# DarlingHang/st-nerf

Hardware: AMD Instinct MI355X
Metric: rendered rays/s (and ray-samples/s) per GPU, 1080p x 128-sample layered render (higher is better)
Workload: dtype f32 (operands split into 3 bf16 pieces, 6 bf16 MFMA terms per product, f32 accumulate); 1 GPU; taekwondo-1080p-64+64; precision=bf16x3, height=1080, width=1920, performer_layers=2, coarse_samples=64, fine_samples=64, parallelism=1 GPU, whole view

## Files before the change

### st-nerf_amd/csrc/mlp_bf16x3.h

```cpp
#pragma once
#include "mlp_common.h"

namespace stnerf {

constexpr int BX_CHUNK = 1024;
constexpr int BX_UNIT = 3 * BX_CHUNK;
constexpr int BX_SLOT = 8 * BX_UNIT;
constexpr int BX_RING = 4;
constexpr int BX_CONST_SPACE = 3072;
constexpr int BX_CONST_MOTION = 1024;
constexpr int BXC_B = 0, BXC_B_DEEP = 1792, BXC_W_SIGMA = 2048, BXC_W_RGB2 = 2304;
constexpr int BXM_B = 0, BXM_W_OUT = 640;

struct BxLayout {
    int64_t f32_floats;
    int64_t consts_off;
    int64_t stream_off;
    int32_t n_slots;
    int64_t total_bytes;
};

__host__ __device__ inline int bx_space_slots(bool deep) {
    return (2 * 4 + 5 * 2 * 16 + 2 * 20 + 16 + (deep ? 16 : 0)) / 2;
}
__host__ __device__ inline int bx_motion_slots() { return (6 + 4 * 8) / 2; }

__host__ __device__ inline BxLayout bx_layout(int kind) {
    BxLayout B;
    const bool space = STNERF_NET_IS_SPACE(kind);
    B.f32_floats = space ? space_layout(STNERF_NET_USES_TIME(kind), STNERF_NET_IS_DEEP(kind)).total : motion_layout().total;
    B.consts_off = (B.f32_floats * 4 + 1023) & ~int64_t(1023);
    B.stream_off = B.consts_off + (space ? BX_CONST_SPACE : BX_CONST_MOTION) * 4;
    B.n_slots = space ? bx_space_slots(STNERF_NET_IS_DEEP(kind)) : bx_motion_slots();
    B.total_bytes = B.stream_off + (int64_t)B.n_slots * BX_SLOT;
    return B;
}

constexpr int BXD_CONST = 1024;
constexpr int BXD_W_SIGMA = 0, BXD_W_RGB2 = 256;
__host__ __device__ inline int bxd_slots(bool with_dpos) { return 8 + 6 * 16 + (with_dpos ? 8 : 0); }

__host__ __device__ inline int bx_kmap_hidden(int t, int h, int j) { return 32 * (t >> 1) + 8 * (2 * (t & 1) + (j >> 2)) + 4 * h + (j & 3); }
__host__ __device__ inline int bx_kmap_enc(int t, int h, int j) { return 16 * t + 8 * h + j; }

struct StageArgs;
struct StoreTapArgs;
struct StageRowsArgs;
int launch_bf16x3_stage_rows(const StageArgs& a, const StageRowsArgs& r, bool deep_rgb, int cus, hipStream_t stream);
int launch_bf16x3_stage(const StageArgs& a, bool deep_rgb, int cus, hipStream_t stream);
int launch_bf16x3_stage_store(const StageArgs& a, const StoreTapArgs& t, int cus, hipStream_t stream);

struct MotionBxArgs {
    const float* net;
    const int32_t* ray_list;
    const int32_t* ray_count;
    int64_t n_rays;
    int32_t ns;
    int32_t flags;
    float* xyz;
    int64_t xyz_ray_stride;
    const float* times;
    int64_t times_ray_stride;
    const int32_t* slots;
    int64_t slot_ray_stride;
    uint32_t* queue;
    int64_t stream_off;
};
int launch_bf16x3_motion(const MotionBxArgs& a, int cus, hipStream_t stream);

}
```

### st-nerf_amd/csrc/mlp_bf16x3_core.h

```cpp
#pragma once
#include <type_traits>

#include "mlp_wave_common.h"
#include "mlp_bf16x3.h"

namespace stnerf {

using bf16x8 = __attribute__((ext_vector_type(8))) __bf16;
using bf16x2 = __attribute__((ext_vector_type(2))) __bf16;
using u32x4 = __attribute__((ext_vector_type(4))) unsigned;

constexpr int BX_LDS_RING = BX_RING * BX_SLOT;
constexpr int BX_LDS_ENC = WV_NW * WV_ENC_FLOATS * 4;
constexpr int BX_LDS_CONST = (BX_CONST_SPACE + BX_CONST_MOTION) * 4;
constexpr int BX_LDS = BX_LDS_RING + BX_LDS_ENC + BX_LDS_CONST + 16 + STNERF_MAX_LAYERS * 8 + (STNERF_MAX_LAYERS + 1) * 4 + 12;
static_assert(BX_LDS <= 160 * 1024, "bf16x3 stage kernel: LDS budget");

#define BX_SB() __builtin_amdgcn_sched_barrier(0)

#ifdef STNERF_BX_PROF
struct BxProf {
    unsigned long long t, acc[16];
};
#define BXP_PARAM , BxProf& bp
// ... 194 lines not shown
        BX_SB();
    }
    if (FIRST && BIG0) {
        const f32x16 z = {0.f, 0.f, 0.f, 0.f, 0.f, 0.f, 0.f, 0.f, 0.f, 0.f, 0.f, 0.f, 0.f, 0.f, 0.f, 0.f};
        big = mfma_bf16(cur.p[0], b0, z);
    } else {
        big = mfma_bf16(cur.p[0], b0, big);
    }
    if (DMA0 >= 0) {
        BX_SB();
        dma_chunk<DMA0 < 0 ? 0 : DMA0 + 2>(*dma);
    }
    if constexpr (!std::is_same<Hook, NoHook>::value) {
        BX_SB();
        hook->template at<U, 2>();
    }
    BX_SB();
}

template <int ST = 0>
__device__ __forceinline__ void slot_turn(Ctx& cx, Dma& d) {
    if constexpr (ST > 0) {
        if (cx.st_on)
            BX_VMCNT(6 + ST);
        else
            BX_VMCNT(6);
    } else {
        BX_VMCNT(6);
    }
    __builtin_amdgcn_s_barrier();
    dma_begin(cx, d);
    BX_SB();
}
__device__ __forceinline__ void slot_done(Ctx& cx) {
    cx.gc += 1;
    cx.rcur = cx.rnext;
    cx.rnext = cx.rnext + (((cx.gc + 1) & (BX_RING - 1)) == 0 ? BX_SLOT - BX_RING * BX_SLOT : BX_SLOT);
}

template <bool FIRST, bool BIG0 = false, class Hook = NoHook, int ST = 0>
__device__ __forceinline__ void slot(Ctx& cx, f32x16 (&big)[4], f32x16 (&small)[4], const bf16x8& k0p0, const bf16x8& k0p1,
                                     const bf16x8& k0p2, const bf16x8& k1p0, const bf16x8& k1p1, const bf16x8& k1p2, Hook* hook = nullptr) {
    unit<0, FIRST, BIG0, -1, Hook>(cx, big[0], small[0], k0p0, k0p1, k0p2, nullptr, hook);
    unit<1, FIRST, BIG0, -1, Hook>(cx, big[1], small[1], k0p0, k0p1, k0p2, nullptr, hook);
    unit<2, FIRST, BIG0, -1, Hook>(cx, big[2], small[2], k0p0, k0p1, k0p2, nullptr, hook);
    unit<3, FIRST, BIG0, -1, Hook>(cx, big[3], small[3], k0p0, k0p1, k0p2, nullptr, hook);
    unit<4, false, false, -1, Hook>(cx, big[0], small[0], k1p0, k1p1, k1p2, nullptr, hook);
    unit<5, false, false, -1, Hook>(cx, big[1], small[1], k1p0, k1p1, k1p2, nullptr, hook);
    Dma d;
    slot_turn<ST>(cx, d);
    unit<6, false, false, 0, Hook>(cx, big[2], small[2], k1p0, k1p1, k1p2, &d, hook);
    unit<7, false, false, 3, Hook>(cx, big[3], small[3], k1p0, k1p1, k1p2, &d, hook);
    slot_done(cx);
}

template <int KS0, int NSLOT, bool FIRST, bool BIG0 = false, int ST = 0>
__device__ __forceinline__ void pass_act(Ctx& cx, f32x16 (&big)[4], f32x16 (&small)[4], const bf16x8 (&act)[3][16]) {
#pragma unroll
    for (int sl = 0; sl < NSLOT; ++sl) {
        const int k = KS0 + 2 * sl;
        if (sl == 0)
            slot<FIRST, BIG0, NoHook, ST>(cx, big, small, act[0][k], act[1][k], act[2][k], act[0][k + 1], act[1][k + 1], act[2][k + 1]);
        else if (sl == 1)
            slot<false, false, NoHook, ST>(cx, big, small, act[0][k], act[1][k], act[2][k], act[0][k + 1], act[1][k + 1], act[2][k + 1]);
        else
            slot<false>(cx, big, small, act[0][k], act[1][k], act[2][k], act[0][k + 1], act[1][k + 1], act[2][k + 1]);
    }
}

__device__ __forceinline__ void load_c(f32x16 (&big)[4], const float* v128, int lane) {
    const float4* b4 = reinterpret_cast<const float4*>(v128) + (lane >> 5);
#pragma unroll
    for (int fb = 0; fb < 4; ++fb)
#pragma unroll
        for (int q = 0; q < 4; ++q) {
            const float4 b = b4[fb * 8 + 2 * q];
            big[fb][4 * q + 0] = b.x;
            big[fb][4 * q + 1] = b.y;
            big[fb][4 * q + 2] = b.z;
            big[fb][4 * q + 3] = b.w;
            BX_SB();
        }
}
__device__ __forceinline__ void load_c_block(f32x16& bigfb, const float* v128, int fb, int lane) {
    const float4* b4 = reinterpret_cast<const float4*>(v128) + (lane >> 5);
#pragma unroll
    for (int q = 0; q < 4; ++q) {
        const float4 b = b4[fb * 8 + 2 * q];
        bigfb[4 * q + 0] = b.x;
        bigfb[4 * q + 1] = b.y;
        bigfb[4 * q + 2] = b.z;
        bigfb[4 * q + 3] = b.w;
    }
}
__device__ __forceinline__ float out_relu(const f32x16& big, const f32x16& small, int i) { return relu_bits(big[i] + small[i]); }

struct Park {
    float v[64];
};
__device__ __forceinline__ void park_put(float& dst, float v) { asm("v_accvgpr_write_b32 %0, %1" : "=a"(dst) : "v"(v)); }
__device__ __forceinline__ float park_get(const float& src) {
    float v;
    asm("v_accvgpr_read_b32 %0, %1" : "=v"(v) : "a"(src));
    return v;
}

// ... 213 lines not shown
    for (int t = 0; t < STEPS; ++t) {
        float v[8];
#pragma unroll
        for (int qq = 0; qq < 2; ++qq) {
            float4 x = make_float4(0.f, 0.f, 0.f, 0.f);
            if (4 * t + 2 + qq < NQ) {
                x = e4[(4 * t + 2 * h + qq) * WV_ROWS + c];
            } else if (4 * t + qq < NQ) {
                const float4 y = e4[(4 * t + qq) * WV_ROWS + c];
                x.x = h == 0 ? y.x : 0.f;
                x.y = h == 0 ? y.y : 0.f;
                x.z = h == 0 ? y.z : 0.f;
                x.w = h == 0 ? y.w : 0.f;
            }
            v[4 * qq + 0] = x.x;
            v[4 * qq + 1] = x.y;
            v[4 * qq + 2] = x.z;
            v[4 * qq + 3] = x.w;
        }
        enc_tap(t, v);
        split8(v, act[0][t], act[1][t], act[2][t]);
        BX_SB();
    }
}

template <int INST = 0>
__device__ __forceinline__ void motion_bx(Ctx& cx, const float* net, const float* cm, float* encw, float (&p)[3], float tv, int flags,
                                          int lane, f32x16 (&big)[4], f32x16 (&small)[4], bf16x8 (&act)[3][16] BXP_PARAM) {
    const MotionLayout L = motion_layout();
    load_c(big, cm + BXM_B, lane);
    encode_motion(encw, lane, p, tv, flags);
    wave_lds_sync();
    enc_to_act<6, WV_ENC_QUADS>(encw, lane, act);
    BXP(BXP_MOTION_ENC);
    pass_act<0, 3, true>(cx, big, small, act);
    BXP(BXP_MOTION_PASS);
#pragma unroll 1
    for (int li = 1; li <= 4; ++li) {
        finish_act<0>(big, small, act, cm + BXM_B + 128 * li, lane);
        BXP(BXP_MOTION_FIN);
        pass_act<0, 4, true>(cx, big, small, act);
        BXP(BXP_MOTION_PASS);
    }
    float fl[3];
    head3(big, small, cm + BXM_W_OUT, net + L.b_out, lane, fl);
#pragma unroll
    for (int c3 = 0; c3 < 3; ++c3) p[c3] = p[c3] + fl[c3];
    BXP(BXP_MOTION_FIN);
}

template <bool DEEP, class Mid, class Tap>
__device__ __forceinline__ float4 space_bx(Ctx& cx, const float* net, const bool use_time, const float* cs, float* encw, const float (&p)[3],
                                           const float* __restrict__ raybias, int32_t ray, int lane, f32x16 (&big)[4], f32x16 (&small)[4],
                                           bf16x8 (&act)[3][16], Mid mid, const Tap& tap BXP_PARAM) {
    const SpaceLayout L = space_layout(use_time, DEEP);
    const int h = lane >> 5;
    constexpr int ST = Tap::on ? BX_TAP_PARK : 0;
    Park pk;
    load_c(big, cs + BXC_B, lane);
    encode_pos(encw, lane, p);
    wave_lds_sync();
    if constexpr (Tap::on) {
        const bool valid = tap_valid(tap, lane);
        float4* dst = reinterpret_cast<float4*>(tap_row(tap, TAP_PE, 4 * h, lane));
        enc_to_act<4, 16>(encw, lane, act, [&](int t, const float (&v)[8]) {
            if (valid) {
                dst[4 * t] = make_float4(v[0], v[1], v[2], v[3]);
                dst[4 * t + 1] = make_float4(v[4], v[5], v[6], v[7]);
            }
        });
    } else {
        enc_to_act<4, 16>(encw, lane, act);
    }
    BXP(BXP_PE);
    pass_act<0, 2, true, false, Tap::on ? BX_TAP_PE : 0>(cx, big, small, act);
    BXP(BXP_PASS);
    finish_park(big, small, pk, cs + BXC_B + 128, lane, tap, 0, 0);
    BXP(BXP_PARK);
    pass_act<0, 2, true, false, ST>(cx, big, small, act);
    BXP(BXP_PASS);
    unpark_act(pk, act);
    BXP(BXP_ACT);
    finish_park(big, small, pk, cs + BXC_B + 256, lane, tap, 0, 128);
    BXP(BXP_PARK);
#define BX_INLINED(call)                           \
    do {                                           \
        if constexpr (Tap::on) {                   \
            [[clang::always_inline]] call;         \
        } else {                                   \
            call;                                  \
        }                                          \
    } while (0)
    auto pe_slots = [&]() {
        const float4* e4 = reinterpret_cast<const float4*>(encw);
#pragma unroll
        for (int sl = 0; sl < 2; ++sl) {
            bf16x8 pe[2][3];
#pragma unroll
            for (int t = 0; t < 2; ++t) {
                float v[8];
#pragma unroll
                for (int qq = 0; qq < 2; ++qq) {
                    const float4 x = e4[(4 * (2 * sl + t) + 2 * h + qq) * WV_ROWS + (lane & 31)];
                    v[4 * qq + 0] = x.x;
                    v[4 * qq + 1] = x.y;
                    v[4 * qq + 2] = x.z;
                    v[4 * qq + 3] = x.w;
                }
                split8(v, pe[t][0], pe[t][1], pe[t][2]);
            }
            slot<false>(cx, big, small, pe[0][0], pe[0][1], pe[0][2], pe[1][0], pe[1][1], pe[1][2]);
        }
    };
    auto layer = [&](int li, auto with_pe) {
        pass_a_unpark<false, ST>(cx, big, small, act, pk);
        pass_act<8, 4, false>(cx, big, small, act);
        if constexpr (decltype(with_pe)::value) BX_INLINED(pe_slots());
        BXP(BXP_PASS);
        finish_park(big, small, pk, cs + BXC_B + 256 * li + 128, lane, tap, li, 0);
        BXP(BXP_PARK);
        pass_b_unpark<ST>(cx, big, small, act, pk);
        if constexpr (decltype(with_pe)::value) BX_INLINED(pe_slots());
        BXP(BXP_PASS);
    };
    auto layer_end = [&](int li) {
        finish_park(big, small, pk, li < 6 ? cs + BXC_B + 256 * (li + 1) : nullptr, lane, tap, li, 128);
        BXP(BXP_PARK);
    };
#pragma unroll 1
    for (int li = 1; li <= 3; ++li) {
        BX_INLINED(layer(li, std::false_type{}));
        BX_INLINED(layer_end(li));
    }
    BX_INLINED(layer(4, std::true_type{}));
    BX_INLINED(layer_end(4));
    float sigma = 0.f;
#pragma unroll 1
    for (int li = 5; li <= 6; ++li) {
        BX_INLINED(layer(li, std::false_type{}));
        if (li == 6) {
            mid();
            sigma = sigma_head(big, small, pk, cs + BXC_W_SIGMA, net[L.b_sigma], lane);
            BXP(BXP_SIGMA);
        }
        BX_INLINED(layer_end(li));
    }
#undef BX_INLINED
    pass_a_unpark<true, ST>(cx, big, small, act, pk);
    pass_act<8, 3, false>(cx, big, small, act);
    BXP(BXP_PASS);
    {
        float4 crow[4][4];
        const float* row = raybias + (int64_t)ray * 128 + 4 * h;
#pragma unroll
        for (int fb = 0; fb < 4; ++fb)
#pragma unroll
            for (int q = 0; q < 4; ++q) crow[fb][q] = *reinterpret_cast<const float4*>(row + fb * 32 + 8 * q);
        pass_act<14, 1, false>(cx, big, small, act);
        BXP(BXP_PASS);
#pragma unroll
        for (int fb = 0; fb < 4; ++fb) {
#pragma unroll
            for (int q = 0; q < 4; ++q) {
                big[fb][4 * q + 0] = (big[fb][4 * q + 0] + small[fb][4 * q + 0]) + crow[fb][q].x;
                big[fb][4 * q + 1] = (big[fb][4 * q + 1] + small[fb][4 * q + 1]) + crow[fb][q].y;
                big[fb][4 * q + 2] = (big[fb][4 * q + 2] + small[fb][4 * q + 2]) + crow[fb][q].z;
                big[fb][4 * q + 3] = (big[fb][4 * q + 3] + small[fb][4 * q + 3]) + crow[fb][q].w;
            }
#pragma unroll
            for (int i = 0; i < 16; ++i) small[fb][i] = 0.f;
            BX_SB();
        }
    }
    if constexpr (Tap::on) finish_park<false>(big, small, pk, nullptr, lane, tap, 7, 0);
    if constexpr (DEEP) {
#pragma unroll 1
        for (int i = 0; i < 2; ++i) {
            finish_act<0>(big, small, act, cs + BXC_B_DEEP + 128 * i, lane);
            pass_act<0, 4, true>(cx, big, small, act);
        }
    }
    float rgb[3];
    head3(big, small, cs + BXC_W_RGB2, net + L.b_rgb2, lane, rgb);
    BXP(BXP_RGB_TAIL);
    return make_float4(rgb[0], rgb[1], rgb[2], sigma);
}

__device__ __forceinline__ void ring_init(Ctx& cx, char* ring, int wave, int lane) {
    cx.ring = ring;
    cx.wave = wave;
    cx.lane = lane;
    cx.gi = 0;
    cx.gc = 0;
    cx.rcur = (uint32_t)(uintptr_t)ring + (uint32_t)lane * 16u;
    cx.rnext = cx.rcur + BX_SLOT;
}
__device__ __forceinline__ void ring_start(Ctx& cx) {
    dma_issue(cx);
    dma_issue(cx);
    dma_issue(cx);
// ... 12 lines not shown
```

### st-nerf_amd/csrc/mlp_bf16x3_stage_kernel.h

```cpp
#pragma once
#include "mlp_bf16x3_core.h"

namespace stnerf {

#ifdef STNERF_BX_PROF
static __device__ unsigned long long g_bxphase[16];
#endif

__device__ __forceinline__ bool tap_wave_stores(const BxStoreTap& tap, const StoreTapArgs& t) {
    return (uint32_t)(tap.wave * WV_ROWS) < tap.nrows && t.bits != nullptr;
}
__device__ __forceinline__ BxNoTap make_bx_tap(const NoTapArgs&, uint32_t, int64_t, int) { return BxNoTap(); }
__device__ __forceinline__ BxNoTap make_bx_tap(const StageRowsArgs&, uint32_t, int64_t, int) { return BxNoTap(); }
__device__ __forceinline__ BxStoreTap make_bx_tap(const StoreTapArgs& t, uint32_t item, int64_t rows, int wave) {
    const int64_t left = rows - (int64_t)item * WV_ITEM;
    return BxStoreTap{&t, item * (uint32_t)WV_ITEM, (uint32_t)(left < WV_ITEM ? left : WV_ITEM), wave};
}

template <bool DEEP, class TapArgs>
__global__ __launch_bounds__(WV_THREADS, 1) void STNERF_STAGE_KERNEL(StageArgs a, TapArgs targs) {
    constexpr bool TAP = std::is_same<TapArgs, StoreTapArgs>::value;
    constexpr bool ROWS = std::is_same<TapArgs, StageRowsArgs>::value;
    extern __shared__ __attribute__((aligned(16))) char smem_bx[];
    const int tid = threadIdx.x;
// ... 122 lines not shown
    }
    Ctx cx;
    ring_init(cx, ring, wave, lane);
    cx.st_on = false;
    segs_of(it0, cx.seg[0], cx.seg[1]);
    segs_of(it1, cx.seg[2], cx.seg[3]);
    cx.idle = cx.seg[1].p;
    ring_start(cx);
    int par = 0;
    f32x16 big[4], small[4];
    bf16x8 act[3][16];
#ifdef STNERF_BX_PROF
    BxProf bp;
    for (int i = 0; i < 16; ++i) bp.acc[i] = 0;
    bp.t = clock64();
#endif
    while (it0 < total) {
        uint32_t pending = 0;
        if (tid == 0) pending = atomicAdd(a.queue, 1u);
        RowRef rr_next;
        uint32_t next_ray = 0;
        if constexpr (TAP) {
            const int64_t row = (int64_t)it1 * WV_ITEM + wave * WV_ROWS + (lane & 31);
            if (row < a.n_rays * a.ns) next_ray = (uint32_t)row / (uint32_t)a.ns;
        } else {
            row_of(it1, rr_next);
        }
        const StageLayer& ly = a.layer[slot_of(it0)];
        {
            const char* sc = reinterpret_cast<const char*>(ly.space) + (sp_kind_stream[ly.use_time ? 1 : 0] - BX_CONST_SPACE * 4) + lane * 16;
            auto d = (__attribute__((address_space(3))) char*)(cs);
#pragma unroll
            for (int i = 0; i < 3; ++i)
                __builtin_amdgcn_global_load_lds(sc + (wave + 4 * i) * BX_CHUNK, (__attribute__((address_space(3))) void*)(d + (wave + 4 * i) * BX_CHUNK), 16, 0, 0);
            if (ly.motion) {
                const char* mc = reinterpret_cast<const char*>(ly.motion) + (mo_stream - BX_CONST_MOTION * 4) + lane * 16;
                auto dm = (__attribute__((address_space(3))) char*)(cm);
                __builtin_amdgcn_global_load_lds(mc + wave * BX_CHUNK, (__attribute__((address_space(3))) void*)(dm + wave * BX_CHUNK), 16, 0, 0);
            }
        }
        float p[3];
#pragma unroll
        for (int c3 = 0; c3 < 3; ++c3) p[c3] = cur.p[c3];
        BX_VMCNT(0);
        __builtin_amdgcn_s_barrier();
        BXP(BXP_TOP);
        int ln = lane;
        asm volatile("" : "+v"(ln));
        if constexpr (!TAP) {
            if (ly.motion) motion_bx(cx, ly.motion, cm, encw, p, cur.tv, ly.motion_flags, ln, big, small, act BXP_ARG);
        }
        const auto tap = make_bx_tap(targs, it0, a.n_rays * a.ns, wave);
        if constexpr (TAP) cx.st_on = tap_wave_stores(tap, targs);
        float4 o = space_bx<DEEP>(cx, ly.space, ly.use_time != 0, cs, encw, p, ly.raybias, cur.ray, ln, big, small, act,
                                  [&]() {
                                      if constexpr (TAP) {
                                          const int64_t row = (int64_t)it1 * WV_ITEM + wave * WV_ROWS + (lane & 31);
                                          rr_next.valid = row < a.n_rays * a.ns;
                                          rr_next.ray = next_ray;
                                          rr_next.k = (int)((uint32_t)row - next_ray * (uint32_t)a.ns);
                                      }
                                      fetch(it1, rr_next, nxt);
                                  }, tap BXP_ARG);
        if constexpr (TAP) {
            const int64_t row = (int64_t)it0 * WV_ITEM + wave * WV_ROWS + (lane & 31);
            cur.raw_off = (int64_t)cur.ray * a.raw_ray_stride + 4 * (row - (int64_t)cur.ray * a.ns);
        }
        if (cur.valid && lane < 32) {
            if (a.sigmoid_rgb) {
                o.x = __builtin_amdgcn_rcpf(1.f + __builtin_amdgcn_exp2f(o.x * -1.44269504088896340736f));
                o.y = __builtin_amdgcn_rcpf(1.f + __builtin_amdgcn_exp2f(o.y * -1.44269504088896340736f));
                o.z = __builtin_amdgcn_rcpf(1.f + __builtin_amdgcn_exp2f(o.z * -1.44269504088896340736f));
            }
            *reinterpret_cast<float4*>(ly.raw + cur.raw_off) = o;
        }
        if (tid == 0) qslot[par] = pending;
        __syncthreads();
        const uint32_t it2 = __builtin_amdgcn_readfirstlane(qslot[par]);
        par ^= 1;
        it0 = it1;
        it1 = it2;
        cur = nxt;
        cx.seg[0] = cx.seg[2];
        cx.seg[1] = cx.seg[3];
        segs_of(it1, cx.seg[2], cx.seg[3]);
        BXP(BXP_END);
#ifdef STNERF_BX_PROF
        bp.acc[BXP_ITEMS] += 1;
#endif
    }
    BX_VMCNT(0);
#ifdef STNERF_BX_PROF
    if (lane == 0)
        for (int i = 0; i < 16; ++i) atomicAdd(&g_bxphase[i], bp.acc[i]);
#endif
}

}
```

### st-nerf_amd/csrc/mlp_stage.h

```cpp
#pragma once
#include <type_traits>

#include "mlp_common.h"

namespace stnerf {

struct StageLayer {
    const float* space;
    const float* motion;
    const int32_t* ray_list;
    const int32_t* ray_count;
    const float* xyz;
    float* raw;
    const float* times;
    int32_t use_time;
    int32_t motion_flags;
    const float* raybias;
};

struct StageArgs {
    StageLayer layer[STNERF_MAX_LAYERS];
    int32_t n_layers, ns;
    int64_t n_rays;
    int64_t xyz_ray_stride, raw_ray_stride, dirs_ray_stride, times_ray_stride;
    const float* dirs;
    uint32_t* queue;
    int32_t sigmoid_rgb;
    float* dbg;
    int32_t dbg_stage;
};

__device__ __forceinline__ int64_t layer_rows(const int32_t* ray_count, int64_t n_rays, int ns) {
    int64_t cnt = n_rays;
    if (ray_count) {
        const int64_t c = *ray_count;
        cnt = c < cnt ? c : cnt;
    }
    return cnt * ns;
}
__device__ __forceinline__ int64_t layer_rows(const StageLayer& ly, int64_t n_rays, int ns) { return layer_rows(ly.ray_count, n_rays, ns); }

struct RowRef {
    int64_t ray;
    int k;
    bool valid;
};
__device__ __forceinline__ RowRef locate_row(const int32_t* ray_list, int64_t row, int64_t rows, int ns) {
    RowRef r{0, 0, row < rows};
    if (r.valid) {
        const int64_t slot = row / ns;
        r.k = (int)(row - slot * ns);
        r.ray = ray_list ? (int64_t)ray_list[slot] : slot;
    }
    return r;
}

__device__ __forceinline__ float lerp_enc(bool frac, float om, float wgt, float va, float vb) {
    return frac ? om * va + wgt * vb : va;
}

struct NoTapArgs {};
constexpr int TAP_PE = 100;
struct StoreTapArgs {
    float* buf[8];
    int32_t ld[8];
    float* pe;
    int32_t ld_pe;
    uint32_t* bits;
    int64_t bits_stride;
};
// ... 23 lines not shown
```

### st-nerf_amd/csrc/pipeline.hip

```cpp
#include <math.h>
#include <stdlib.h>
#include <string.h>

#include "common.h"
#include "mlp_bf16x3.h"

using namespace stnerf;

namespace {

struct Carve {
    char* base;
    int64_t off, cap;
    template <class T>
    T* take(int64_t count) {
        off = (off + 255) & ~int64_t(255);
        T* p = reinterpret_cast<T*>(base + off);
        off += count * (int64_t)sizeof(T);
        return p;
    }
};

struct Plan {
    int64_t t_c, xyz_c, raw_c, w_c, slots, t_f, xyz_f, raw_f, list, count, flags, raybias;
// ... 336 lines not shown
            STNERF_REQUIRE(((uintptr_t)e.raw_coarse & 15) == 0 && (p->only_coarse || ((uintptr_t)e.raw_fine & 15) == 0),
                           "render_rays: layer cache buffers of layer %d must be 16-byte aligned", i);
            STNERF_REQUIRE(e.capacity >= 0, "render_rays: layer cache entry %d with a negative capacity", i);
            (e.mode == STNERF_LAYER_CACHE_REUSE ? lreuse : lcap) |= 1u << i;
        }
    }
    call->lcap = lcap;
    call->lreuse = lreuse;
    call->term = 0;
    if (flagged && !p->only_coarse)
        for (int i = 0; i < l; ++i)
            if (o.terminate[i] && (i == 0 ? cache_mode == STNERF_BKGD_CACHE_OFF : p->shown[i] != 0 && !((lcap | lreuse) >> i & 1))) call->term |= 1u << i;
    if (o.occ) {
        const int orc = check_occupancy_table(o.occ, l, "render_rays");
        if (orc) return orc;
        STNERF_REQUIRE(((uintptr_t)o.counts & 7) == 0, "render_rays: occupancy counts must be 8-byte aligned");
    }
    return STNERF_OK;
}

int launch_sequence(RENDER_PARAMS, const stnerf_render_options& o, const Call& c, const Plan& pl, const Workspace& w, stnerf_stream_t stream) {
    const int l = p->l, n1 = p->n1, n2 = p->n2, S = n1 + n2, rs = p->ray_stride;
    const bool cached = c.cache_mode == STNERF_BKGD_CACHE_REUSE;
    const uint32_t lcap = c.lcap, lreuse = c.lreuse, term = c.term;
    const int64_t row_cap = c.rows.row_cap;
    hipStream_t st = as_stream(stream);
    int rc;

    rc = stnerf_sample_coarse_rot(rays, n, rs, boxes, box_ray_stride, l, n1, jitter, p->seed, p->ray_index_base,
                                  p->ray_index_stripe, p->ray_index_period,
                                  p->has_edits ? p->edits_coarse : nullptr, p->pivot, o.rot, w.t_c, w.xyz_c, mask, stream);
    if (rc) return rc;
    if (o.occ) {
        rc = stnerf_occupancy_cull(w.xyz_c, n, l, n1, o.occ, mask, o.counts, stream);
        if (rc) return rc;
    }
    if (hipMemsetAsync(w.ray_count, 0, sizeof(int32_t) * pl.count, st) != hipSuccess) {
        set_error("render_rays: hipMemsetAsync failed");
        return STNERF_ELAUNCH;
    }
    rc = stnerf_compact_rays(mask, n, l, w.ray_list, w.ray_count, stream);
    if (rc) return rc;

    uint32_t reuse = 0;
    if (p->precision == 3 && !p->only_coarse && p->use_deform_time) {
        const char* sw = getenv("STNERF_MOTION_REUSE");
        if (!(sw && sw[0] == '0'))
            for (int i = 1; i < l; ++i)
                if (p->shown[i] && !w.row_list[i] && !(lreuse >> i & 1) && (!p->has_edits || memcmp(&p->edits_coarse[i], &p->edits_fine[i], sizeof(stnerf_layer_edit)) == 0))
                    reuse |= 1u << i;
    }
    uint32_t* motion_queue = reinterpret_cast<uint32_t*>(w.ray_count + STNERF_MAX_LAYERS + 2);

    auto stage = [&](float* xyz, float* raw, int ns, bool fine, uint32_t moved) -> int {
        const int64_t xs = (int64_t)l * ns * 3, ws_ = (int64_t)l * ns * 4;
        if (p->precision == 0 || p->precision == 3) {
            stnerf_stage_layer sl[STNERF_MAX_LAYERS];
            stnerf_stage_rows sr[STNERF_MAX_LAYERS];
            memset(sr, 0, sizeof(sr));
            int ns_l = 0;
            bool any_list = false;
            for (int pass = 0; pass < 2; ++pass) {
                for (int i = cached ? 1 : 0; i < l; ++i) {
                    if (i > 0 && (!p->shown[i] || (lreuse >> i & 1))) continue;
                    const bool deform = i == 0 ? p->bkgd_use_deform_time != 0 : p->use_deform_time != 0;
                    if ((pass == 0) != deform) continue;
                    const bool timed = (i > 0 ? 1 : p->bkgd_use_space_time) && p->use_space_time;
                    stnerf_stage_layer& e = sl[ns_l++];
                    e.space = i == 0 ? (fine ? nets->bkgd_fine : nets->bkgd) : (fine ? nets->space_fine[i] : nets->space[i]);
                    e.motion = deform && !(moved >> i & 1) ? nets->motion[i] : nullptr;
                    e.ray_list = i == 0 ? nullptr : w.ray_list + (int64_t)i * n;
                    e.ray_count = i == 0 ? nullptr : w.ray_count + i;
                    e.xyz = xyz + (int64_t)i * ns * 3;
                    e.raw = raw + (int64_t)i * ns * 4;
                    e.times = (timed || deform) ? rays + (p->retiming ? 6 + i : 6) : nullptr;
                    e.use_time = timed ? 1 : 0;
                    e.motion_flags = i == 0 ? STNERF_MOTION_PLAIN_TIME : 0;
                    e.rotation = o.rot ? o.rot + i : nullptr;
                    const bool culled = o.samples && o.samples[i];
                    if (i == 0 && c.bg) {
                        const bool stop = fine && (term & 1);
                        const int r1 = stnerf_background_rows(n, e.xyz, xs, ns, o.bkgd_grid, stop ? w.t_f : nullptr, (int64_t)l * ns, stop ? w.t_stop : nullptr,
                                                              e.raw, ws_, w.row_list[0], row_cap, w.row_count, o.bkgd_counts, stream);
                        if (r1) return r1;
                    } else if (fine && (term >> i & 1)) {
                        const int r1 = stnerf_visibility_rows(e.ray_list, e.ray_count, n, i, e.xyz, xs, w.t_f + (int64_t)i * ns, (int64_t)l * ns, w.t_stop, ns,
                                                              culled ? o.occ + i : nullptr, e.raw, ws_, w.row_list[i], row_cap, w.row_count + i,
                                                              o.visibility_counts, stream);
                        if (r1) return r1;
                    } else if (culled) {
                        const int r1 = stnerf_occupancy_rows(e.ray_list, e.ray_count, n, i, e.xyz, xs, ns, o.occ + i, e.raw, ws_, w.row_list[i], row_cap,
                                                             w.row_count + i, o.sample_counts, stream);
                        if (r1) return r1;
                    } else {
                        continue;
                    }
                    sr[ns_l - 1].row_list = w.row_list[i];
                    sr[ns_l - 1].row_count = w.row_count + i;
                    any_list = true;
                }
            }
            if (ns_l == 0) return STNERF_OK;
            set_launch_tag(fine ? 1 : 0);
            const int r2 = stnerf_mlp_stage_rows(sl, any_list ? sr : nullptr, ns_l, n, ns, rays + 3, rs, rs, xs, ws_,
                                                 (p->deep_rgb ? STNERF_STAGE_DEEP_RGB : 0) | STNERF_STAGE_SIGMOID_RGB | (p->precision == 3 ? STNERF_STAGE_BF16X3 : 0),
                                                 reinterpret_cast<uint32_t*>(w.ray_count + STNERF_MAX_LAYERS + (fine ? 1 : 0)), w.ray_bias, stream);
            set_launch_tag(-1);
            return r2;
        }
        for (int i = cached ? 1 : 0; i < l; ++i) {
            if (i == 0 ? !p->bkgd_use_deform_time : !p->use_deform_time) continue;
            if (i > 0 && (!p->shown[i] || (lreuse >> i & 1))) continue;
            set_launch_tag(i);
            const float* times = rays + (p->retiming ? 6 + i : 6);
            const int32_t* lst = i == 0 ? nullptr : w.ray_list + (int64_t)i * n;
            const int32_t* cnt = i == 0 ? nullptr : w.ray_count + i;
            const int flags = STNERF_MOTION_ADD_TO_XYZ | (i == 0 ? STNERF_MOTION_PLAIN_TIME : 0);
            const int r2 = stnerf_motionnet_fwd(nets->motion[i], n, ns, lst, cnt, xyz + (int64_t)i * ns * 3, xs, times,
                                                      rs, nullptr, 0, flags, stream);
            if (r2) return r2;
        }
        for (int i = cached ? 1 : 0; i < l; ++i) {
            if (i > 0 && (!p->shown[i] || (lreuse >> i & 1))) continue;
            set_launch_tag(i);
            const void* net = i == 0 ? (fine ? nets->bkgd_fine : nets->bkgd) : (fine ? nets->space_fine[i] : nets->space[i]);
            const bool timed = (i > 0 ? 1 : p->bkgd_use_space_time) && p->use_space_time;
            const int kind = timed ? (p->deep_rgb ? STNERF_NET_SPACE_TIME_DEEP : STNERF_NET_SPACE_TIME)
                                   : (p->deep_rgb ? STNERF_NET_SPACE_DEEP : STNERF_NET_SPACE);
            const float* times = timed ? rays + (p->retiming ? 6 + i : 6) : nullptr;
            const int32_t* lst = i == 0 ? nullptr : w.ray_list + (int64_t)i * n;
            const int32_t* cnt = i == 0 ? nullptr : w.ray_count + i;
            const int r2 = stnerf_spacenet_fwd_rot(kind, net, n, ns, lst, cnt, xyz + (int64_t)i * ns * 3, xs, rays + 3, rs, times, rs,
                                                   raw + (int64_t)i * ns * 4, ws_, w.ray_bias + (int64_t)i * n * 128, o.rot ? o.rot + i : nullptr,
                                                   stream);
            if (r2) return r2;
        }
        set_launch_tag(-1);
        return STNERF_OK;
    };
    for (int i = 1; i < l; ++i) {
        if (!(reuse >> i & 1)) continue;
        rc = motion_rows(nets, p, rays, n, i, n1, n1, w.xyz_c, w.ray_list, w.ray_count, nullptr, 0, motion_queue + 2 * i, st);
        if (rc) return rc;
    }
    auto stage_and_cache = [&](float* xyz, float* raw, int ns, bool fine, float* kept) -> int {
        const int r2 = stage(xyz, raw, ns, fine, reuse);
        if (r2) return r2;
        if (c.cache_mode != STNERF_BKGD_CACHE_OFF) {
            set_launch_tag(0);
            const int r3 = stnerf_copy_layer_raw(raw, n, l, 0, ns, kept, c.cache_mode == STNERF_BKGD_CACHE_CAPTURE, stream);
            set_launch_tag(-1);
            if (r3) return r3;
        }
        for (int i = 1; i < l; ++i) {
            if (!((lcap | lreuse) >> i & 1)) continue;
            const stnerf_layer_cache& e = o.layers[i];
            const bool capture = lcap >> i & 1;
            const int32_t* lst = capture && fine ? e.rays : w.ray_list + (int64_t)i * n;
            const int32_t* cnt = capture && fine ? e.count : w.ray_count + i;
// ... 168 lines not shown
```

### st-nerf_amd/csrc/stage_entry.hip

```cpp
#include <string.h>

#include "mlp_wave_core.h"
#include "mlp_bf16x3.h"

using namespace stnerf;

namespace stnerf {
struct MotionOpTap : NoTap {
    float* flow_out;
    float* xyz_out;
    float p[3];
    __device__ __forceinline__ void flow(const float (&fl)[3], int lane) const {
        if (lane >= 32) return;
        if (flow_out) {
            flow_out[0] = fl[0];
            flow_out[1] = fl[1];
            flow_out[2] = fl[2];
        }
        if (xyz_out) {
            xyz_out[0] = p[0] + fl[0];
            xyz_out[1] = p[1] + fl[1];
            xyz_out[2] = p[2] + fl[2];
        }
    }
};
struct MotionOpArgs {
    const float* net;
    const int32_t* ray_list;
    const int32_t* ray_count;
    int64_t n_rays;
    int32_t ns;
    int32_t flags;
    float* xyz;
    int64_t xyz_ray_stride;
    const float* times;
    int64_t times_ray_stride;
    float* flow;
    int64_t flow_ray_stride;
    __device__ __forceinline__ int64_t row_count() const { return layer_rows(ray_count, n_rays, ns); }
    __device__ __forceinline__ MotionOpTap fetch(int64_t row, int64_t n, float (&p)[3], float& tv) const {
        const RowRef r = locate_row(ray_list, row, n, ns);
        MotionOpTap t{{}, nullptr, nullptr, {0.f, 0.f, 0.f}};
        tv = 0.f;
        if (r.valid) {
            float* src = xyz + r.ray * xyz_ray_stride + 3 * r.k;
#pragma unroll
            for (int c3 = 0; c3 < 3; ++c3) t.p[c3] = src[c3];
            tv = times[r.ray * times_ray_stride];
            if (flow) t.flow_out = flow + r.ray * flow_ray_stride + 3 * r.k;
            if (flags & STNERF_MOTION_ADD_TO_XYZ) t.xyz_out = src;
        }
#pragma unroll
        for (int c3 = 0; c3 < 3; ++c3) p[c3] = t.p[c3];
        return t;
    }
};
}

extern "C" int stnerf_mlp_stage(const stnerf_stage_layer* layers, int n_layers, int64_t n_rays, int ns, const float* dirs,
                                int64_t dirs_ray_stride, int64_t times_ray_stride, int64_t xyz_ray_stride,
                                int64_t raw_ray_stride, int flags, uint32_t* queue, float* ray_bias, stnerf_stream_t stream) {
    return stnerf_mlp_stage_rows(layers, nullptr, n_layers, n_rays, ns, dirs, dirs_ray_stride, times_ray_stride, xyz_ray_stride, raw_ray_stride,
                                 flags, queue, ray_bias, stream);
}

extern "C" int stnerf_mlp_stage_rows(const stnerf_stage_layer* layers, const stnerf_stage_rows* rows, int n_layers, int64_t n_rays, int ns,
                                     const float* dirs, int64_t dirs_ray_stride, int64_t times_ray_stride, int64_t xyz_ray_stride,
                                     int64_t raw_ray_stride, int flags, uint32_t* queue, float* ray_bias, stnerf_stream_t stream) {
    STNERF_REQUIRE(layers && dirs && queue && ray_bias, "mlp_stage: null pointer");
    STNERF_REQUIRE(((uintptr_t)ray_bias & 15) == 0, "mlp_stage: ray_bias must be 16-byte aligned");
    STNERF_REQUIRE(n_layers >= 1 && n_layers <= STNERF_MAX_LAYERS && n_rays >= 0 && ns >= 1, "mlp_stage: bad shape");
    STNERF_REQUIRE((raw_ray_stride & 3) == 0, "mlp_stage: raw ray stride must be a multiple of 4 floats");
    STNERF_REQUIRE((flags & ~(STNERF_STAGE_DEEP_RGB | STNERF_STAGE_SIGMOID_RGB | STNERF_STAGE_BF16X3)) == 0, "mlp_stage: unknown flags %d", flags);
    StageRowsArgs ra;
    memset(&ra, 0, sizeof(ra));
    bool listed = false;
    for (int i = 0; rows && i < n_layers; ++i) {
        if (!rows[i].row_list) continue;
        STNERF_REQUIRE(rows[i].row_count, "mlp_stage: layer %d: a row list without its row count", i);
        STNERF_REQUIRE(ns <= 256 && n_rays <= ((int64_t)1 << 23), "mlp_stage: a row list packs (ray << 8 | k): ns <= 256 and n_rays <= 2^23 (got %d, %lld)",
                       ns, (long long)n_rays);
        ra.row_list[i] = rows[i].row_list;
        ra.row_count[i] = rows[i].row_count;
        listed = true;
    }
    if (n_rays == 0) return STNERF_OK;
    const int deep_rgb = (flags & STNERF_STAGE_DEEP_RGB) != 0;
    const bool bf16x3 = (flags & STNERF_STAGE_BF16X3) != 0;
    StageArgs a;
    memset(&a, 0, sizeof(a));
    a.sigmoid_rgb = (flags & STNERF_STAGE_SIGMOID_RGB) != 0;
    LaunchTimer timer(PROF_MLP_STAGE, deep_rgb | (bf16x3 ? 2 : 0) | (listed ? 4 : 0), n_rays, ns, 0, as_stream(stream));
    for (int i = 0; i < n_layers; ++i) {
        const stnerf_stage_layer& s = layers[i];
        STNERF_REQUIRE(s.space && s.xyz && s.raw, "mlp_stage: layer %d: null pointer", i);
        const uintptr_t amask = bf16x3 ? 1023 : 15;
        STNERF_REQUIRE(((uintptr_t)s.space & amask) == 0 && ((uintptr_t)s.raw & 15) == 0 && (!s.motion || ((uintptr_t)s.motion & amask) == 0),
                       "mlp_stage: layer %d: packed weights must be %d-byte aligned, raw 16-byte aligned", i, (int)amask + 1);
        STNERF_REQUIRE(!(s.use_time || s.motion) || s.times, "mlp_stage: layer %d needs its frame-id column", i);
        a.layer[i] = StageLayer{static_cast<const float*>(s.space), static_cast<const float*>(s.motion), s.ray_list,
                                s.ray_count, s.xyz, s.raw, s.times, s.use_time, s.motion_flags,
                                ray_bias + (int64_t)i * n_rays * 128};
        const int kind = s.use_time ? (deep_rgb ? STNERF_NET_SPACE_TIME_DEEP : STNERF_NET_SPACE_TIME)
                                    : (deep_rgb ? STNERF_NET_SPACE_DEEP : STNERF_NET_SPACE);
        if (const int rc = launch_ray_bias(kind, static_cast<const float*>(s.space), n_rays, s.ray_list, s.ray_count, dirs,
                                           dirs_ray_stride, s.times, times_ray_stride, ray_bias + (int64_t)i * n_rays * 128,
                                           as_stream(stream), s.rotation))
            return rc;
    }
    a.n_layers = n_layers;
    a.ns = ns;
    a.n_rays = n_rays;
    a.xyz_ray_stride = xyz_ray_stride;
    a.raw_ray_stride = raw_ray_stride;
    a.dirs_ray_stride = dirs_ray_stride;
    a.times_ray_stride = times_ray_stride;
    a.dirs = dirs;
    a.queue = queue;
    int dev = 0, cus = 256;
    if (hipGetDevice(&dev) == hipSuccess) (void)hipDeviceGetAttribute(&cus, hipDeviceAttributeMultiprocessorCount, dev);
    if (listed)
        return bf16x3 ? launch_bf16x3_stage_rows(a, ra, deep_rgb != 0, cus, as_stream(stream))
                      : launch_wave_stage_rows(a, ra, deep_rgb != 0, cus, as_stream(stream));
    return bf16x3 ? launch_bf16x3_stage(a, deep_rgb != 0, cus, as_stream(stream)) : launch_wave_stage(a, deep_rgb != 0, cus, as_stream(stream));
}

extern "C" int stnerf_spacenet_fwd(int kind, const void* packed, int64_t n_rays, int ns, const int32_t* ray_list,
                                   const int32_t* ray_count, const float* xyz, int64_t xyz_ray_stride,
                                   const float* dirs, int64_t dirs_ray_stride, const float* times,
                                   int64_t times_ray_stride, float* raw, int64_t raw_ray_stride, float* ray_bias,
                                   stnerf_stream_t stream) {
    return stnerf_spacenet_fwd_rot(kind, packed, n_rays, ns, ray_list, ray_count, xyz, xyz_ray_stride, dirs, dirs_ray_stride, times,
                                   times_ray_stride, raw, raw_ray_stride, ray_bias, nullptr, stream);
}

extern "C" int stnerf_spacenet_fwd_rot(int kind, const void* packed, int64_t n_rays, int ns, const int32_t* ray_list,
                                       const int32_t* ray_count, const float* xyz, int64_t xyz_ray_stride,
                                       const float* dirs, int64_t dirs_ray_stride, const float* times,
                                       int64_t times_ray_stride, float* raw, int64_t raw_ray_stride, float* ray_bias,
                                       const stnerf_layer_rotation* rotation_host, stnerf_stream_t stream) {
    STNERF_REQUIRE(STNERF_NET_IS_SPACE(kind), "spacenet_fwd: bad kind %d", kind);
    STNERF_REQUIRE(packed && xyz && dirs && raw && ray_bias, "spacenet_fwd: null pointer");
    STNERF_REQUIRE(((uintptr_t)ray_bias & 15) == 0, "spacenet_fwd: ray_bias must be 16-byte aligned");
    STNERF_REQUIRE(!STNERF_NET_USES_TIME(kind) || times, "spacenet_fwd: net takes time but times is null");
    STNERF_REQUIRE(n_rays >= 0 && ns >= 1, "spacenet_fwd: bad shape n_rays=%lld ns=%d", (long long)n_rays, ns);
    STNERF_REQUIRE((raw_ray_stride & 3) == 0 && ((uintptr_t)raw & 15) == 0, "spacenet_fwd: raw must be 16-byte aligned");
    STNERF_REQUIRE(((uintptr_t)packed & 15) == 0, "spacenet_fwd: packed weights must be 16-byte aligned");
    if (n_rays == 0) return STNERF_OK;
    if (const int rc = launch_ray_bias(kind, static_cast<const float*>(packed), n_rays, ray_list, ray_count, dirs, dirs_ray_stride,
                                       times, times_ray_stride, ray_bias, as_stream(stream), rotation_host))
        return rc;
    StageArgs a;
    memset(&a, 0, sizeof(a));
    a.layer[0] = StageLayer{static_cast<const float*>(packed), nullptr, ray_list, ray_count, xyz, raw, times,
                            STNERF_NET_USES_TIME(kind) ? 1 : 0, 0, ray_bias};
// ... 29 lines not shown
```

Baseline: 696,600 rays/s.

## Skip RGB head MLP for waves whose samples all have non-positive density

After the density layers, each wave ballots whether any valid sample has positive sigma. If none does, and the layer's compositing weight cannot make such samples matter, the RGB-branch MFMA passes are skipped. The kernel still drains the weight DMA ring with idle slots so the streaming schedule stays in step. Skipping avoids a large share of matrix work for empty space but relies on zero-sigma samples contributing nothing, outputs zero RGB for those rows, and adds a wave-level branch.

```diff
diff --git a/st-nerf_amd/csrc/mlp_bf16x3.h b/st-nerf_amd/csrc/mlp_bf16x3.h
--- a/st-nerf_amd/csrc/mlp_bf16x3.h
+++ b/st-nerf_amd/csrc/mlp_bf16x3.h
@@ -50,6 +50,10 @@
 int launch_bf16x3_stage(const StageArgs& a, bool deep_rgb, int cus, hipStream_t stream);
 int launch_bf16x3_stage_store(const StageArgs& a, const StoreTapArgs& t, int cus, hipStream_t stream);
 
+int mlp_stage_rows_skip_dead(const stnerf_stage_layer* layers, const stnerf_stage_rows* rows, int n_layers, int64_t n_rays, int ns,
+                             const float* dirs, int64_t dirs_ray_stride, int64_t times_ray_stride, int64_t xyz_ray_stride,
+                             int64_t raw_ray_stride, int flags, uint32_t* queue, float* ray_bias, uint32_t skip_dead_rgb, stnerf_stream_t stream);
+
 struct MotionBxArgs {
     const float* net;
     const int32_t* ray_list;
diff --git a/st-nerf_amd/csrc/mlp_bf16x3_core.h b/st-nerf_amd/csrc/mlp_bf16x3_core.h
--- a/st-nerf_amd/csrc/mlp_bf16x3_core.h
+++ b/st-nerf_amd/csrc/mlp_bf16x3_core.h
@@ -270,6 +270,37 @@
     unit<6, false, false, 0, Hook>(cx, big[2], small[2], k1p0, k1p1, k1p2, &d, hook);
     unit<7, false, false, 3, Hook>(cx, big[3], small[3], k1p0, k1p1, k1p2, &d, hook);
     slot_done(cx);
+}
+
+template <bool LAST>
+__device__ __forceinline__ void slot_idle(Ctx& cx) {
+    Dma d;
+    slot_turn(cx, d);
+    dma_chunk<0>(d);
+    dma_chunk<1>(d);
+    dma_chunk<2>(d);
+    dma_chunk<3>(d);
+    dma_chunk<4>(d);
+    dma_chunk<5>(d);
+    if (LAST) {
+        a_read<0>(cx.A[0].p[0], cx.rnext);
+        a_read<BX_CHUNK>(cx.A[0].p[1], cx.rnext);
+        a_read<2 * BX_CHUNK>(cx.A[0].p[2], cx.rnext);
+        a_read<BX_UNIT>(cx.A[1].p[0], cx.rnext);
+        a_read<BX_UNIT + BX_CHUNK>(cx.A[1].p[1], cx.rnext);
+        a_read<BX_UNIT + 2 * BX_CHUNK>(cx.A[1].p[2], cx.rnext);
+    }
+    BX_SB();
+    slot_done(cx);
+}
+template <int NSLOT>
+__device__ __forceinline__ void slots_idle(Ctx& cx) {
+    a_wait<0>(cx.A[0]);
+    a_wait<0>(cx.A[1]);
+    BX_SB();
+#pragma unroll 1
+    for (int sl = 0; sl < NSLOT - 1; ++sl) slot_idle<false>(cx);
+    slot_idle<true>(cx);
 }
 
 template <int KS0, int NSLOT, bool FIRST, bool BIG0 = false, int ST = 0>
@@ -589,7 +620,8 @@
 template <bool DEEP, class Mid, class Tap>
 __device__ __forceinline__ float4 space_bx(Ctx& cx, const float* net, const bool use_time, const float* cs, float* encw, const float (&p)[3],
                                            const float* __restrict__ raybias, int32_t ray, int lane, f32x16 (&big)[4], f32x16 (&small)[4],
-                                           bf16x8 (&act)[3][16], Mid mid, const Tap& tap BXP_PARAM) {
+                                           bf16x8 (&act)[3][16], Mid mid, const Tap& tap, const bool skip_dead, const bool valid,
+                                           bool& dead BXP_PARAM) {
     const SpaceLayout L = space_layout(use_time, DEEP);
     const int h = lane >> 5;
     constexpr int ST = Tap::on ? BX_TAP_PARK : 0;
@@ -683,6 +715,15 @@
         BX_INLINED(layer_end(li));
     }
 #undef BX_INLINED
+    dead = false;
+    if constexpr (!Tap::on) {
+        if (skip_dead) dead = __builtin_amdgcn_ballot_w64(valid && !(sigma <= 0.f)) == 0ull;
+    }
+    if (dead) {
+        slots_idle<8 + (DEEP ? 8 : 0)>(cx);
+        BXP(BXP_RGB_TAIL);
+        return make_float4(0.f, 0.f, 0.f, sigma);
+    }
     pass_a_unpark<true, ST>(cx, big, small, act, pk);
     pass_act<8, 3, false>(cx, big, small, act);
     BXP(BXP_PASS);
diff --git a/st-nerf_amd/csrc/mlp_bf16x3_stage_kernel.h b/st-nerf_amd/csrc/mlp_bf16x3_stage_kernel.h
--- a/st-nerf_amd/csrc/mlp_bf16x3_stage_kernel.h
+++ b/st-nerf_amd/csrc/mlp_bf16x3_stage_kernel.h
@@ -198,6 +198,7 @@
         }
         const auto tap = make_bx_tap(targs, it0, a.n_rays * a.ns, wave);
         if constexpr (TAP) cx.st_on = tap_wave_stores(tap, targs);
+        bool dead;
         float4 o = space_bx<DEEP>(cx, ly.space, ly.use_time != 0, cs, encw, p, ly.raybias, cur.ray, ln, big, small, act,
                                   [&]() {
                                       if constexpr (TAP) {
@@ -207,13 +208,13 @@
                                           rr_next.k = (int)((uint32_t)row - next_ray * (uint32_t)a.ns);
                                       }
                                       fetch(it1, rr_next, nxt);
-                                  }, tap BXP_ARG);
+                                  }, tap, !TAP && ly.skip_dead_rgb != 0, cur.valid, dead BXP_ARG);
         if constexpr (TAP) {
             const int64_t row = (int64_t)it0 * WV_ITEM + wave * WV_ROWS + (lane & 31);
             cur.raw_off = (int64_t)cur.ray * a.raw_ray_stride + 4 * (row - (int64_t)cur.ray * a.ns);
         }
         if (cur.valid && lane < 32) {
-            if (a.sigmoid_rgb) {
+            if (a.sigmoid_rgb && !dead) {
                 o.x = __builtin_amdgcn_rcpf(1.f + __builtin_amdgcn_exp2f(o.x * -1.44269504088896340736f));
                 o.y = __builtin_amdgcn_rcpf(1.f + __builtin_amdgcn_exp2f(o.y * -1.44269504088896340736f));
                 o.z = __builtin_amdgcn_rcpf(1.f + __builtin_amdgcn_exp2f(o.z * -1.44269504088896340736f));
diff --git a/st-nerf_amd/csrc/mlp_stage.h b/st-nerf_amd/csrc/mlp_stage.h
--- a/st-nerf_amd/csrc/mlp_stage.h
+++ b/st-nerf_amd/csrc/mlp_stage.h
@@ -16,6 +16,7 @@
     int32_t use_time;
     int32_t motion_flags;
     const float* raybias;
+    int32_t skip_dead_rgb;
 };
 
 struct StageArgs {
diff --git a/st-nerf_amd/csrc/pipeline.hip b/st-nerf_amd/csrc/pipeline.hip
--- a/st-nerf_amd/csrc/pipeline.hip
+++ b/st-nerf_amd/csrc/pipeline.hip
@@ -412,6 +412,15 @@
     }
     uint32_t* motion_queue = reinterpret_cast<uint32_t*>(w.ray_count + STNERF_MAX_LAYERS + 2);
 
+    const char* sd = getenv("STNERF_SKIP_DEAD_RGB");
+    const bool skip_dead = !(sd && sd[0] == '0');
+    auto dead_weighs_nothing = [&](int i, bool fine) {
+        if (!fine) return true;
+        if ((lcap >> i & 1) && i == 2) return false;
+        const float factor = o.layer_alpha ? o.layer_alpha[i] : (l > 2 && i == 2 ? p->alpha : 1.f);
+        return factor >= 0.f;
+    };
+
     auto stage = [&](float* xyz, float* raw, int ns, bool fine, uint32_t moved) -> int {
         const int64_t xs = (int64_t)l * ns * 3, ws_ = (int64_t)l * ns * 4;
         if (p->precision == 0 || p->precision == 3) {
@@ -419,6 +428,7 @@
             stnerf_stage_rows sr[STNERF_MAX_LAYERS];
             memset(sr, 0, sizeof(sr));
             int ns_l = 0;
+            uint32_t skip_mask = 0;
             bool any_list = false;
             for (int pass = 0; pass < 2; ++pass) {
                 for (int i = cached ? 1 : 0; i < l; ++i) {
@@ -427,6 +437,7 @@
                     if ((pass == 0) != deform) continue;
                     const bool timed = (i > 0 ? 1 : p->bkgd_use_space_time) && p->use_space_time;
                     stnerf_stage_layer& e = sl[ns_l++];
+                    if (skip_dead && dead_weighs_nothing(i, fine)) skip_mask |= 1u << (ns_l - 1);
                     e.space = i == 0 ? (fine ? nets->bkgd_fine : nets->bkgd) : (fine ? nets->space_fine[i] : nets->space[i]);
                     e.motion = deform && !(moved >> i & 1) ? nets->motion[i] : nullptr;
                     e.ray_list = i == 0 ? nullptr : w.ray_list + (int64_t)i * n;
@@ -462,9 +473,9 @@
             }
             if (ns_l == 0) return STNERF_OK;
             set_launch_tag(fine ? 1 : 0);
-            const int r2 = stnerf_mlp_stage_rows(sl, any_list ? sr : nullptr, ns_l, n, ns, rays + 3, rs, rs, xs, ws_,
-                                                 (p->deep_rgb ? STNERF_STAGE_DEEP_RGB : 0) | STNERF_STAGE_SIGMOID_RGB | (p->precision == 3 ? STNERF_STAGE_BF16X3 : 0),
-                                                 reinterpret_cast<uint32_t*>(w.ray_count + STNERF_MAX_LAYERS + (fine ? 1 : 0)), w.ray_bias, stream);
+            const int r2 = mlp_stage_rows_skip_dead(sl, any_list ? sr : nullptr, ns_l, n, ns, rays + 3, rs, rs, xs, ws_,
+                                                    (p->deep_rgb ? STNERF_STAGE_DEEP_RGB : 0) | STNERF_STAGE_SIGMOID_RGB | (p->precision == 3 ? STNERF_STAGE_BF16X3 : 0),
+                                                    reinterpret_cast<uint32_t*>(w.ray_count + STNERF_MAX_LAYERS + (fine ? 1 : 0)), w.ray_bias, skip_mask, stream);
             set_launch_tag(-1);
             return r2;
         }
diff --git a/st-nerf_amd/csrc/stage_entry.hip b/st-nerf_amd/csrc/stage_entry.hip
--- a/st-nerf_amd/csrc/stage_entry.hip
+++ b/st-nerf_amd/csrc/stage_entry.hip
@@ -67,6 +67,14 @@
 extern "C" int stnerf_mlp_stage_rows(const stnerf_stage_layer* layers, const stnerf_stage_rows* rows, int n_layers, int64_t n_rays, int ns,
                                      const float* dirs, int64_t dirs_ray_stride, int64_t times_ray_stride, int64_t xyz_ray_stride,
                                      int64_t raw_ray_stride, int flags, uint32_t* queue, float* ray_bias, stnerf_stream_t stream) {
+    return mlp_stage_rows_skip_dead(layers, rows, n_layers, n_rays, ns, dirs, dirs_ray_stride, times_ray_stride, xyz_ray_stride, raw_ray_stride,
+                                    flags, queue, ray_bias, 0u, stream);
+}
+
+int stnerf::mlp_stage_rows_skip_dead(const stnerf_stage_layer* layers, const stnerf_stage_rows* rows, int n_layers, int64_t n_rays, int ns,
+                                     const float* dirs, int64_t dirs_ray_stride, int64_t times_ray_stride, int64_t xyz_ray_stride,
+                                     int64_t raw_ray_stride, int flags, uint32_t* queue, float* ray_bias, uint32_t skip_dead_rgb,
+                                     stnerf_stream_t stream) {
     STNERF_REQUIRE(layers && dirs && queue && ray_bias, "mlp_stage: null pointer");
     STNERF_REQUIRE(((uintptr_t)ray_bias & 15) == 0, "mlp_stage: ray_bias must be 16-byte aligned");
     STNERF_REQUIRE(n_layers >= 1 && n_layers <= STNERF_MAX_LAYERS && n_rays >= 0 && ns >= 1, "mlp_stage: bad shape");
@@ -100,7 +108,7 @@
         STNERF_REQUIRE(!(s.use_time || s.motion) || s.times, "mlp_stage: layer %d needs its frame-id column", i);
         a.layer[i] = StageLayer{static_cast<const float*>(s.space), static_cast<const float*>(s.motion), s.ray_list,
                                 s.ray_count, s.xyz, s.raw, s.times, s.use_time, s.motion_flags,
-                                ray_bias + (int64_t)i * n_rays * 128};
+                                ray_bias + (int64_t)i * n_rays * 128, bf16x3 && (skip_dead_rgb >> i & 1u) ? 1 : 0};
         const int kind = s.use_time ? (deep_rgb ? STNERF_NET_SPACE_TIME_DEEP : STNERF_NET_SPACE_TIME)
                                     : (deep_rgb ? STNERF_NET_SPACE_DEEP : STNERF_NET_SPACE);
         if (const int rc = launch_ray_bias(kind, static_cast<const float*>(s.space), n_rays, s.ray_list, s.ray_count, dirs,
```

Measured after the change: 697,800 rays/s (median of 6 runs). No clear change (+0.2%).
